# panshengyi/MemVul

Measured on AMD Instinct MI355X. Metric: issue-reports/sec at seq_len=256 (BERT-base issue encoder + 124-anchor memory match), higher is better.
Workload: dtype fp16 + fp8 (MV_F16X8: fp16 MFMA sweep + one OCP-e4m3 MFMA correction sweep per GEMM, fp32 accumulate); 1 GPU; BASELINE.json configs[1]: 1xMI355X-per-rank, bert-base-uncased geometry (12 layers), seq_len=256, batch=256, 124-anchor CWE memory, compute dtype MV_F16X8; seeded random-init weights, synthetic token ids resident in HBM; compute=precise, global_batch=256, seq_len=256, anchors=124, parallelism=dp1 (corpus shards, one all-gather of (score,label) stats), stats_transport=none (one rank)

## Files before the change

### memvul_amd/build.py

```python
from __future__ import annotations

import os
import shutil
import subprocess
from struct import error as struct_error
import sys

HERE = os.path.dirname(os.path.abspath(__file__))
ROOT = os.path.dirname(HERE)
CSRC = os.path.join(HERE, "csrc")
LIB_DIR = os.path.join(HERE, "lib")
LIB_PATH = os.path.join(LIB_DIR, "libmemvul_hip.so")
LIB_PATH_DEV = os.path.join(LIB_DIR, "libmemvul_hip_dev.so")
DEV_FLAGS = ("-DMEMVUL_DEV_SWITCHES",)
SOURCES = ["engine.hip"]
HEADERS = ["common.h", "gemm.h", "gemm_pp.h", "attention.h", "attention_v2.h", "misc_kernels.h", "match_topk.h", "ref_f32.h", "sink_census.h", "route.h", os.path.join(ROOT, "include", "memvul_hip.h")]
ARCH = "gfx950"


def hipcc_path() -> str:
    for c in (os.environ.get("HIPCC"), shutil.which("hipcc"), "/opt/rocm/bin/hipcc"):
        if c and os.path.exists(c):
            return c
    raise RuntimeError("hipcc not found (need ROCm at /opt/rocm)")


STAMP_PATH = LIB_PATH + ".stamp"


def _paths(dev: bool):
    lib = LIB_PATH_DEV if dev else LIB_PATH
    return lib, lib + ".stamp"
FLAGS = ["-O3", "-std=c++17", "-fPIC", "-shared", "-fno-gpu-rdc", "-Wall", "-Wno-unused-function", "-Wno-unused-value"]


def _compiler_id():
    try:
        return subprocess.run([hipcc_path(), "--version"], capture_output=True, check=True).stdout
    except Exception:
        return None


def source_fingerprint(extra_flags=()) -> str:
    import hashlib

    h = hashlib.sha256()
    h.update(" ".join([ARCH, *FLAGS, *extra_flags]).encode())
    deps = [os.path.join(CSRC, s) for s in SOURCES] + [h_ if os.path.isabs(h_) else os.path.join(CSRC, h_) for h_ in HEADERS]
    for d in deps:
        h.update(os.path.basename(d).encode())
        with open(d, "rb") as f:
            h.update(f.read())
    return h.hexdigest()


def build_fingerprint(extra_flags=()) -> str:
    import hashlib

    cc = _compiler_id()
    return "src %s\ncc %s" % (source_fingerprint(extra_flags), hashlib.sha256(cc).hexdigest() if cc is not None else "unknown")


def device_code_objects(lib_path: str = None) -> list:
    import struct

    data = open(lib_path or LIB_PATH, "rb").read()
    magic = b"__CLANG_OFFLOAD_BUNDLE__"
    found = []
    i = data.find(magic)
# ... 92 lines not shown
```

### memvul_amd/csrc/attention.h

```cpp
#pragma once
#include "common.h"

struct AttnArgs {
  const half_t* q;
  const half_t* k;
  const half_t* vt;
  const int32_t* lens;
  half_t* ctx;
  int S;
  int B;
  uint8_t* ctx8;
  unsigned long long* x8_sat;
  const half_t* vt_lo;
  const half_t *q_lo, *k_lo;
  const half_t* vlo_sp;
  unsigned long long* conc;
  int lo8_min_len;
  half_t* sp_lo_out;
  uint32_t* seq_over;
};
#define MV_SINK_COLLISION 0.25f

template <bool LO = false>
__global__ __launch_bounds__(256) void attention_cls_kernel(const float* __restrict__ q, const half_t* __restrict__ k,
                                                            const half_t* __restrict__ vt, const int32_t* __restrict__ lens,
                                                            half_t* __restrict__ ctx, int S, int nbh, float* __restrict__ ctx32 = nullptr,
                                                            const half_t* __restrict__ vlo_sp = nullptr, const half_t* __restrict__ k_lo = nullptr,
                                                            const half_t* __restrict__ vt_lo = nullptr) {
  __shared__ float ps[4][512];
  const int lane = threadIdx.x & 63, wave = threadIdx.x >> 6;
  const int bh = blockIdx.x * 4 + wave;
  if (bh >= nbh) return;
  const int b = bh / MV_HEADS, h = bh - b * MV_HEADS;
  const int len = lens[b];
  const int c = lane & 7, sub = lane >> 3;
  float* pw = ps[wave];
  float qv[8];
  {
    const float4* qp = (const float4*)(q + (size_t)b * MV_HIDDEN + h * MV_HEAD_DIM + 8 * c);
    const float4 t0 = qp[0], t1 = qp[1];
    qv[0] = (float)(half_t)t0.x; qv[1] = (float)(half_t)t0.y; qv[2] = (float)(half_t)t0.z; qv[3] = (float)(half_t)t0.w;
    qv[4] = (float)(half_t)t1.x; qv[5] = (float)(half_t)t1.y; qv[6] = (float)(half_t)t1.z; qv[7] = (float)(half_t)t1.w;
    if constexpr (LO) { qv[0] = t0.x; qv[1] = t0.y; qv[2] = t0.z; qv[3] = t0.w; qv[4] = t1.x; qv[5] = t1.y; qv[6] = t1.z; qv[7] = t1.w; }
  }
  const half_t* kb = k + (size_t)bh * S * MV_HEAD_DIM + (size_t)sub * MV_HEAD_DIM + 8 * c;
#pragma unroll 8
  for (int key0 = 0; key0 < S; key0 += 8) {
    const half8_t kk = *(const half8_t*)(kb + (size_t)key0 * MV_HEAD_DIM);
    float s = 0.f;
#pragma unroll
    for (int e = 0; e < 8; ++e) s = __builtin_fmaf(qv[e], (float)kk[e], s);
    if constexpr (LO) {
      const half8_t kl = *(const half8_t*)(k_lo + (kb - k) + (size_t)key0 * MV_HEAD_DIM);
      float sl = 0.f;
#pragma unroll
      for (int e = 0; e < 8; ++e) sl = __builtin_fmaf(qv[e], (float)kl[e], sl);
      s += sl;
    }
    s += __shfl_xor(s, 1, 64);
    s += __shfl_xor(s, 2, 64);
    s += __shfl_xor(s, 4, 64);
    if (c == 0) pw[key0 + sub] = s + ((key0 + sub >= len) ? -10000.0f : 0.0f);
  }
  __builtin_amdgcn_wave_barrier();
  float mx = -3.0e38f;
  for (int key = lane; key < S; key += 64) mx = fmaxf(mx, pw[key]);
  mx = wave_max(mx);
  float psum = 0.f;
  for (int key = lane; key < S; key += 64) {
    const float p = __expf(pw[key] - mx);
    psum += p;
    pw[key] = LO ? p : (float)(half_t)p;
  }
  const float inv = 1.0f / wave_sum(psum);
  __builtin_amdgcn_wave_barrier();
  float acc[8];
#pragma unroll
  for (int db = 0; db < 8; ++db) acc[db] = 0.f;
  const half_t* vb = vt + ((size_t)bh * MV_HEAD_DIM + sub) * S + 8 * c;
  for (int kb0 = 0; kb0 < S; kb0 += 64) {
    const float4 p0 = *(const float4*)(pw + kb0 + 8 * c), p1 = *(const float4*)(pw + kb0 + 8 * c + 4);
    const float pr[8] = {p0.x, p0.y, p0.z, p0.w, p1.x, p1.y, p1.z, p1.w};
#pragma unroll
    for (int db = 0; db < 8; ++db) {
      const half8_t vv = *(const half8_t*)(vb + (size_t)(8 * db) * S + kb0);
#pragma unroll
      for (int e = 0; e < 8; ++e) acc[db] = __builtin_fmaf(pr[e], (float)vv[e], acc[db]);
    }
  }
  if constexpr (LO) {
    float accl[8];
#pragma unroll
    for (int db = 0; db < 8; ++db) accl[db] = 0.f;
    const half_t* vlb = vt_lo + (vb - vt);
    for (int kb0 = 0; kb0 < S; kb0 += 64) {
      const float4 p0 = *(const float4*)(pw + kb0 + 8 * c), p1 = *(const float4*)(pw + kb0 + 8 * c + 4);
      const float pr[8] = {p0.x, p0.y, p0.z, p0.w, p1.x, p1.y, p1.z, p1.w};
#pragma unroll
      for (int db = 0; db < 8; ++db) {
        const half8_t vv = *(const half8_t*)(vlb + (size_t)(8 * db) * S + kb0);
#pragma unroll
        for (int e = 0; e < 8; ++e) accl[db] = __builtin_fmaf(pr[e], (float)vv[e], accl[db]);
      }
    }
#pragma unroll
    for (int db = 0; db < 8; ++db) acc[db] += accl[db];
  }
  float out = 0.f;
#pragma unroll
  for (int db = 0; db < 8; ++db) {
    float t = acc[db];
    t += __shfl_xor(t, 1, 64);
    t += __shfl_xor(t, 2, 64);
    t += __shfl_xor(t, 4, 64);
    out = (c == db) ? t : out;
  }
  if (vlo_sp) {
    const half2_t l2 = *(const half2_t*)(vlo_sp + ((size_t)bh * MV_HEAD_DIM + 8 * c + sub) * 2);
    out = __builtin_fmaf(__builtin_fmaf(pw[0], (float)l2[0], pw[1] * (float)l2[1]), 1.0f / 2048.0f, out);
  }
  if (ctx32) ctx32[(size_t)b * MV_HIDDEN + h * MV_HEAD_DIM + 8 * c + sub] = out * inv;
  else ctx[(size_t)b * MV_HIDDEN + h * MV_HEAD_DIM + 8 * c + sub] = (half_t)(out * inv);
}
```

### memvul_amd/csrc/engine.hip

```cpp
#include <hip/hip_runtime.h>
#include <dlfcn.h>
#include <rccl/rccl.h>
#include <unistd.h>

#include <algorithm>
#include <charconv>
#include <chrono>
#include <cmath>
#include <cstdio>
#include <cstdlib>
#include <cstring>
#include <map>
#include <string>
#include <vector>

#include "../../include/memvul_hip.h"
#include "common.h"
#include "gemm.h"
#include "gemm_pp.h"
#include "attention.h"
#include "attention_v2.h"
#include "misc_kernels.h"
#include "match_topk.h"
#include "ref_f32.h"
#include "sink_census.h"
#include "route.h"

namespace {

enum KernelClass {
  KC_EMBED_LN = 0, KC_GEMM_QKV, KC_ATTENTION, KC_GEMM_OUT, KC_LN, KC_GEMM_FFN1, KC_GEMM_FFN2,
  KC_POOL_HEAD, KC_MATCH, KC_TOPK, KC_TEST_GEMM, KC_CLS_ROW_TERM, KC_GEMM_KV_LAST, KC_CLS_TAIL
};
const char* kKernelClassNames[MV_NUM_KERNEL_CLASSES] = {
    "embed_ln", "gemm_qkv", "attention", "gemm_attn_out", "layernorm", "gemm_ffn1_gelu", "gemm_ffn2",
    "pool_head", "match", "topk", "test_gemm", "cls_row_term", "gemm_kv_last", "cls_tail"};

thread_local std::string g_create_error;

struct HostTensor {
  std::vector<float> data;
  std::vector<int64_t> shape;
};

struct LayerW {
  half_t *wqkv = nullptr, *wo = nullptr, *w1 = nullptr, *w2 = nullptr;
  float *bqkv = nullptr, *bo = nullptr, *b1 = nullptr, *b2 = nullptr;
  half_t *wqkv_f = nullptr, *w1_f = nullptr;
  float *bqkv_f = nullptr, *b1_f = nullptr;
  uint8_t *wqkv_f8 = nullptr, *wo8 = nullptr, *w1_f8 = nullptr, *w28 = nullptr;
  int sc_qkv = 0, sc_o = 0, sc_1 = 0, sc_2 = 0;
  float *wqT32 = nullptr, *woT32 = nullptr, *w1T32 = nullptr, *w2T32 = nullptr;
  float *wqkv32 = nullptr, *wo32 = nullptr, *w132 = nullptr, *w232 = nullptr;
  float *ln1g = nullptr, *ln1b = nullptr, *ln2g = nullptr, *ln2b = nullptr;
};

inline int64_t round_up(int64_t x, int64_t m) { return (x + m - 1) / m * m; }

inline uint16_t f32_to_f16_bits(float f) {
  uint32_t x;
  std::memcpy(&x, &f, 4);
  const uint32_t sign = (x >> 16) & 0x8000u;
  x &= 0x7fffffffu;
  if (x >= 0x7f800000u) return (uint16_t)(sign | 0x7c00u | ((x > 0x7f800000u) ? 0x200u : 0));
  if (x >= 0x477ff000u) return (uint16_t)(sign | 0x7c00u);
  if (x < 0x38800000u) {
    if (x < 0x33000000u) return (uint16_t)sign;
    const int e = (int)(x >> 23);
    uint32_t m = (x & 0x7fffffu) | 0x800000u;
    const int shift = 126 - e;
    const uint32_t half_m = m >> shift;
    const uint32_t rem = m & ((1u << shift) - 1), halfway = 1u << (shift - 1);
    uint32_t r = half_m;
    if (rem > halfway || (rem == halfway && (half_m & 1))) r++;
    return (uint16_t)(sign | r);
  }
  const uint32_t e = (x >> 23) - 112, m = x & 0x7fffffu;
  uint32_t h = (e << 10) | (m >> 13);
  const uint32_t rem = m & 0x1fffu;
  if (rem > 0x1000u || (rem == 0x1000u && (h & 1))) h++;
  return (uint16_t)(sign | h);
}
inline float f16_bits_to_f32(uint16_t h) {
  const uint32_t sign = (uint32_t)(h & 0x8000u) << 16;
  uint32_t e = (h >> 10) & 0x1f, m = h & 0x3ffu, x;
  if (e == 0) {
    if (m == 0) x = sign;
    else {
      int sh = 0;
      while (!(m & 0x400u)) { m <<= 1; sh++; }
      m &= 0x3ffu;
      x = sign | ((uint32_t)(113 - sh) << 23) | (m << 13);
    }
  } else if (e == 31) x = sign | 0x7f800000u | (m << 13);
  else x = sign | ((e + 112) << 23) | (m << 13);
  float f;
  std::memcpy(&f, &x, 4);
  return f;
}
inline float bf16_bits_to_f32(uint16_t h) {
  uint32_t x = (uint32_t)h << 16;
  float f;
  std::memcpy(&f, &x, 4);
  return f;
}
// ... 509 lines not shown
                       wk.tile_both);
    if (int rc = launch_check(h, "cls_tile_flags")) return rc;
  }
  const bool special = big && x8;
  auto row_term = [&](const half_t* A, const half_t* W, int N, int K) -> int {
    ProfScope ps(h, wk.stream, KC_CLS_ROW_TERM);
    GemmArgs t{};
    t.M = (int)round_up(2 * B, 64); t.Mreal = 2 * B; t.S = 64; t.A = A; t.W = W; t.N = N; t.K = K; t.outf = wk.cls_corr;
    t.GN = choose_gn(N / 64, 8);
    hipLaunchKernelGGL((gemm_ring_kernel<EPI_F32, 1, 1, 2, 2, 64, 4, 2>), dim3((unsigned)((t.M / 64) * (N / 64))), dim3(256), RING64_LDS, wk.stream, t);
    return launch_check(h, "row term gemm_ring");
  };
  const unsigned ln_grid = (unsigned)((M + 3) / 4);
  {
    ProfScope ps(h, wk.stream, KC_EMBED_LN);
    if (big)
      hipLaunchKernelGGL(embed_ln_kernel<true>, dim3(ln_grid), dim3(256), 0, wk.stream, d_ids, pitch, S_in, Sp, (int)M, c.vocab_size,
                         h->wemb, h->pemb, h->temb, h->embg, h->embb, c.ln_eps, wk.xres, wk.x16, wk.lnstats,
                         x8 ? (half_t*)nullptr : wk.xlo, x8 ? wk.x8 : (uint8_t*)nullptr, h->x8_sat, special ? d_lens : (const int32_t*)nullptr,
                         special ? wk.st_lo : (half_t*)nullptr);
    else
      hipLaunchKernelGGL(embed_ln_kernel<false>, dim3(ln_grid), dim3(256), 0, wk.stream, d_ids, pitch, S_in, Sp, (int)M, c.vocab_size,
                         h->wemb, h->pemb, h->temb, h->embg, h->embb, c.ln_eps, wk.xres, wk.x16, (float*)nullptr,
                         (half_t*)nullptr, (uint8_t*)nullptr, (unsigned long long*)nullptr);
    if (int rc = launch_check(h, "embed_ln")) return rc;
  }
  const float *pend_g = h->embg, *pend_b = h->embb;
  auto run_ln = [&](float* x32, half_t* x16, int rows, const float* g, const float* b) -> int {
    ProfScope ps(h, wk.stream, KC_LN);
    hipLaunchKernelGGL(ln_kernel<true>, dim3((unsigned)((rows + 3) / 4)), dim3(256), 0, wk.stream, x32, x16, rows, g, b, c.ln_eps,
                       (float*)nullptr);
    return launch_check(h, "layernorm");
  };
  auto final_ln = [&](const float* g, const float* b) -> int {
    const size_t n4 = (size_t)M * MV_HIDDEN / 4;
    hipLaunchKernelGGL(hilo_to_f32_kernel, dim3((unsigned)((n4 + 255) / 256)), dim3(256), 0, wk.stream, wk.x16, wk.xlo, n4, wk.xres,
                       special ? (const half_t*)wk.st_lo : (const half_t*)nullptr, Sp, (const uint8_t*)wk.x8);
    if (int rc = launch_check(h, "hilo_to_f32")) return rc;
    return run_ln(wk.xres, wk.x16, (int)M, g, b);
  };
  if (big && n_layers == 0) { if (int rc = final_ln(h->embg, h->embb)) return rc; }
  float *st_in = wk.lnstats, *st_mid = wk.lnpart;
  for (int l = 0; l < n_layers; ++l) {
    const LayerW& w = h->L[l];
    const bool last = (l == n_layers - 1);
    GemmArgs g{};
    g.M = (int)Mpad; g.Mreal = (int)M; g.S = Sp; g.ln_eps = c.ln_eps; g.x8_sat = h->x8_sat;
    g.tile_both = (cls_as && one_seq_tiles) ? wk.tile_both : nullptr;
    g.q = wk.q; g.k = wk.k; g.vt = wk.vt;
    const half_t* wqkv = big ? w.wqkv_f : w.wqkv;
    const float* bqkv = big ? w.bqkv_f : w.bqkv;
    if (last && prune) {
      const int Bp = (int)round_up(B, 128);
      g.A = wk.x16; g.W = wqkv + (size_t)MV_HIDDEN * MV_HIDDEN; g.bias = bqkv + MV_HIDDEN; g.N = 2 * MV_HIDDEN; g.K = MV_HIDDEN;
      g.col0 = MV_HIDDEN;
      if (big) {
        g.lnstats = st_in;
        if (x8) { g.A8 = wk.x8; g.W8 = w.wqkv_f8 + (size_t)MV_HIDDEN * 2 * MV_HIDDEN; g.x8_scale = w.sc_qkv; g.x8_terms = 3; g.x8_aside_mask = qkv_mask; }
        if (special) {
          if ((qkv_mask & 6) != 6) {
            if (int rc = row_term(wk.st_lo, g.W, g.N, g.K)) return rc;
            g.cls_corr = wk.cls_corr;
          }
          g.vlo_sp = two_plane ? nullptr : wk.vlo_sp;
        }
        if (safe) { g.vt_lo = wk.vt_lo; g.q_lo = wk.q_lo; g.k_lo = wk.k_lo; }
        if (int rc = launch_pp<PP_QK>(h, wk.stream, KC_GEMM_KV_LAST, g)) return rc;
      } else if (int rc = launch_small<EPI_QKV>(h, wk.stream, KC_GEMM_KV_LAST, g)) return rc;
      ProfScope tail(h, wk.stream, KC_CLS_TAIL);
      const uint32_t keep_mask = h->prof_mask;
      h->prof_mask = 0;
      auto tail_rc = [&]() -> int {
        hipLaunchKernelGGL(cls_gather_kernel, dim3((B + 3) / 4), dim3(256), 0, wk.stream, wk.xres, wk.x16, Sp, B,
                           big ? st_in : (const float*)nullptr, pend_g, pend_b, wk.c32, wk.c16, big ? 1 : 0,
                           (big && !x8) ? wk.xlo : (const half_t*)nullptr, big ? 1 : 0, c.ln_eps, special ? (const half_t*)wk.st_lo : (const half_t*)nullptr);
        if (int rc = launch_check(h, "cls_gather")) return rc;
        if (x8) {
          const unsigned gx = (unsigned)((B + 31) / 32);
          hipLaunchKernelGGL((dense768_kernel<2, MV_HIDDEN>), dim3(gx, MV_HIDDEN / 32), dim3(512), 0, wk.stream, (const float*)wk.c32,
                             (size_t)MV_HIDDEN, B, (const float*)w.wqT32, (const float*)w.bqkv, MV_HIDDEN, wk.cq, (const float*)nullptr);
          if (int rc = launch_check(h, "cls q")) return rc;
          if (safe)
            hipLaunchKernelGGL(attention_cls_kernel<true>, dim3((B * MV_HEADS + 3) / 4), dim3(256), 0, wk.stream, wk.cq, wk.k, wk.vt, d_lens, wk.cctx, Sp,
                               B * MV_HEADS, wk.pooled, (const half_t*)g.vlo_sp, (const half_t*)wk.k_lo, (const half_t*)wk.vt_lo);
          else
            hipLaunchKernelGGL(attention_cls_kernel<false>, dim3((B * MV_HEADS + 3) / 4), dim3(256), 0, wk.stream, wk.cq, wk.k, wk.vt, d_lens, wk.cctx, Sp,
                               B * MV_HEADS, wk.pooled, (const half_t*)g.vlo_sp, (const half_t*)nullptr, (const half_t*)nullptr);
          if (int rc = launch_check(h, "attention_cls")) return rc;
          hipLaunchKernelGGL((dense768_kernel<4, MV_HIDDEN>), dim3(gx, MV_HIDDEN / 32), dim3(512), 0, wk.stream, (const float*)wk.pooled,
                             (size_t)MV_HIDDEN, B, (const float*)w.woT32, (const float*)w.bo, MV_HIDDEN, wk.c32, (const float*)wk.c32);
          if (int rc = launch_check(h, "cls out")) return rc;
          if (int rc = run_ln(wk.c32, wk.c16, B, w.ln1g, w.ln1b)) return rc;
          hipLaunchKernelGGL((dense768_kernel<3, MV_HIDDEN>), dim3(gx, MV_INTER / 32), dim3(512), 0, wk.stream, (const float*)wk.c32,
                             (size_t)MV_HIDDEN, B, (const float*)w.w1T32, (const float*)w.b1, MV_INTER, wk.ch32, (const float*)nullptr);
          if (int rc = launch_check(h, "cls ffn1")) return rc;
          hipLaunchKernelGGL((dense768_kernel<4, MV_INTER>), dim3(gx, MV_HIDDEN / 32), dim3(512), 0, wk.stream, (const float*)wk.ch32,
                             (size_t)MV_INTER, B, (const float*)w.w2T32, (const float*)w.b2, MV_HIDDEN, wk.c32, (const float*)wk.c32);
          if (int rc = launch_check(h, "cls ffn2")) return rc;
          if (int rc = run_ln(wk.c32, wk.c16, B, w.ln2g, w.ln2b)) return rc;
          return pool_head(h, wk, wk.c32, MV_HIDDEN, B, u_out);
        }
        GemmArgs t{};
        t.M = Bp; t.Mreal = B; t.S = 64;
        t.A = wk.c16; t.W = w.wqkv; t.bias = w.bqkv; t.N = MV_HIDDEN; t.K = MV_HIDDEN; t.outf = wk.cq;
        if (int rc = launch_small<EPI_F32>(h, wk.stream, KC_CLS_TAIL, t)) return rc;
        hipLaunchKernelGGL(attention_cls_kernel<false>, dim3((B * MV_HEADS + 3) / 4), dim3(256), 0, wk.stream, wk.cq, wk.k, wk.vt,
                           d_lens, wk.cctx, Sp, B * MV_HEADS, (float*)nullptr, (const half_t*)nullptr, (const half_t*)nullptr, (const half_t*)nullptr);
        if (int rc = launch_check(h, "attention_cls")) return rc;
        t.A = wk.cctx; t.W = w.wo; t.bias = w.bo; t.N = MV_HIDDEN; t.K = MV_HIDDEN; t.xres = wk.c32; t.outf = nullptr;
        if (int rc = launch_small<EPI_RES>(h, wk.stream, KC_CLS_TAIL, t)) return rc;
        if (int rc = run_ln(wk.c32, wk.c16, B, w.ln1g, w.ln1b)) return rc;
        t.A = wk.c16; t.W = w.w1; t.bias = w.b1; t.N = MV_INTER; t.K = MV_HIDDEN; t.out16 = wk.ch16;
        if (int rc = launch_small<EPI_GELU>(h, wk.stream, KC_CLS_TAIL, t)) return rc;
        t.A = wk.ch16; t.W = w.w2; t.bias = w.b2; t.N = MV_HIDDEN; t.K = MV_INTER; t.xres = wk.c32;
        if (int rc = launch_small<EPI_RES>(h, wk.stream, KC_CLS_TAIL, t)) return rc;
        if (int rc = run_ln(wk.c32, wk.c16, B, w.ln2g, w.ln2b)) return rc;
        return pool_head(h, wk, wk.c32, MV_HIDDEN, B, u_out);
      }();
      h->prof_mask = keep_mask;
      return tail_rc;
    }
    if (big) {
      g.A = wk.x16; g.W = wqkv; g.bias = bqkv; g.N = 3 * MV_HIDDEN; g.K = MV_HIDDEN; g.lnstats = st_in;
      if (x8) { g.A8 = wk.x8; g.W8 = w.wqkv_f8; g.x8_scale = w.sc_qkv; g.x8_terms = 3; g.x8_aside_mask = qkv_mask; }
      g.vt_lo = two_plane ? wk.vt_lo : nullptr;
      g.q_lo = wk.q_lo; g.k_lo = wk.k_lo;
      if (special) {
        if (qkv_mask != 7) {
          if (int rc = row_term(wk.st_lo, g.W, g.N, g.K)) return rc;
          g.cls_corr = wk.cls_corr;
        }
        g.vlo_sp = g.vt_lo ? nullptr : wk.vlo_sp;
      }
      if (int rc = launch_pp<PP_QK>(h, wk.stream, KC_GEMM_QKV, g)) return rc;
      g.cls_corr = nullptr; g.vlo_sp = nullptr;
      if (h->census && x8 && pf.monitor) {
        ProfScope ps(h, wk.stream, KC_ATTENTION);
        hipLaunchKernelGGL(sink_census_kernel, dim3((unsigned)((B * MV_HEADS + 3) / 4)), dim3(256), 0, wk.stream, (const half_t*)wk.q, (const half_t*)wk.k, d_lens,
                           d_ids, pitch, S_in, Sp, B * MV_HEADS, c.vocab_size, h->census_items, h->census_share, h->census_heads + (size_t)l * MV_HEADS);
        if (int rc = launch_check(h, "sink_census")) return rc;
      }
      if (int rc = launch_attention(h, wk, d_lens, B, Sp, x8, cls_as, pf)) return rc;
      g.A = wk.ctx; g.W = w.wo; g.bias = w.bo; g.N = MV_HIDDEN; g.K = MV_HIDDEN;
      g.lnstats = st_in; g.lng = pend_g; g.lnb = pend_b; g.lnpart = st_mid; g.out16 = wk.x16; g.out16b = wk.xlo;
      if (x8) { g.A8 = wk.ctx8; g.W8 = w.wo8; g.x8_scale = w.sc_o; g.out8 = wk.x8; g.x8_terms = 2; }
      if (cls_as) {
        if (int rc = row_term(wk.cls_lo, g.W, g.N, g.K)) return rc;
        g.cls_corr = wk.cls_corr; g.x8_terms = 1;
        g.out8_hi_only = 0;
      }
      if (special) g.sp_lo_out = wk.st_lo;
      if (int rc = launch_pp<PP_RESLN3>(h, wk.stream, KC_GEMM_OUT, g)) return rc;
      pend_g = w.ln1g; pend_b = w.ln1b;
      g.A = wk.x16; g.W = w.w1_f; g.bias = w.b1_f; g.N = MV_INTER; g.K = MV_HIDDEN; g.lnstats = st_mid; g.out16 = wk.h16;
      g.out16b = nullptr; g.lnpart = nullptr; g.sp_lo_out = nullptr;
      if (x8) { g.A8 = wk.x8; g.W8 = w.w1_f8; g.x8_scale = w.sc_1; g.out8 = wk.h8; g.x8_terms = 2; }
      if (cls_as) {
        if (int rc = row_term(wk.st_lo, g.W, g.N, g.K)) return rc;
        g.x8_terms = 1;
        g.out8_hi_only = 1;
// ... 845 lines not shown
        pack[(size_t)(2 * H + i)] = t3->data[(size_t)i];
      }
      if ((rc = upload_f32(h, s0, &w.bqkv, pack.data(), 3 * H))) return rc;
      bqkv_host = pack;
    }
    if (!f32) {
      const std::string lnk = l == 0 ? P + "embeddings.LayerNorm." : P + "encoder.layer." + std::to_string(l - 1) + ".output.LayerNorm.";
      const HostTensor *tg = nullptr, *tb = nullptr;
      if ((rc = need(h, lnk + "weight", {H}, &tg))) return rc;
      if ((rc = need(h, lnk + "bias", {H}, &tb))) return rc;
      std::vector<float> Wf, bf;
      fold_layernorm(wqkv_host.data(), bqkv_host.data(), tg->data.data(), tb->data.data(), 3 * H, H, Wf, bf);
      if ((rc = upload_f16(h, s0, &w.wqkv_f, Wf.data(), 3 * H * H))) return rc;
      if (precise && (rc = upload_x8_weight(h, s0, &w.wqkv_f8, &w.sc_qkv, Wf.data(), 3 * H, H))) return rc;
      if ((rc = upload_f32(h, s0, &w.bqkv_f, bf.data(), 3 * H))) return rc;
    }
    NEED(q + "attention.output.dense.weight", H, H);
    if (f32 && (rc = upload_f32(h, s0, &w.wo32, t->data.data(), H * H))) return rc;
    if (!f32 && (rc = upload_f16(h, s0, &w.wo, t->data.data(), H * H))) return rc;
    if (precise && (rc = upload_x8_weight(h, s0, &w.wo8, &w.sc_o, t->data.data(), H, H))) return rc;
    NEED(q + "attention.output.dense.bias", H);
    if ((rc = upload_f32(h, s0, &w.bo, t->data.data(), H))) return rc;
    NEED(q + "attention.output.LayerNorm.weight", H);
    if ((rc = upload_f32(h, s0, &w.ln1g, t->data.data(), H))) return rc;
    NEED(q + "attention.output.LayerNorm.bias", H);
    if ((rc = upload_f32(h, s0, &w.ln1b, t->data.data(), H))) return rc;
    NEED(q + "intermediate.dense.weight", I, H);
    if (f32 && (rc = upload_f32(h, s0, &w.w132, t->data.data(), I * H))) return rc;
    if (!f32 && (rc = upload_f16(h, s0, &w.w1, t->data.data(), I * H))) return rc;
    NEED(q + "intermediate.dense.bias", I);
    if ((rc = upload_f32(h, s0, &w.b1, t->data.data(), I))) return rc;
    if (!f32) {
      const HostTensor *tw = nullptr, *tg = nullptr, *tb = nullptr;
      if ((rc = need(h, q + "intermediate.dense.weight", {I, H}, &tw))) return rc;
      if ((rc = need(h, q + "attention.output.LayerNorm.weight", {H}, &tg))) return rc;
      if ((rc = need(h, q + "attention.output.LayerNorm.bias", {H}, &tb))) return rc;
      std::vector<float> Wf, bf;
      fold_layernorm(tw->data.data(), t->data.data(), tg->data.data(), tb->data.data(), I, H, Wf, bf);
      if ((rc = upload_f16(h, s0, &w.w1_f, Wf.data(), I * H))) return rc;
      if (precise && (rc = upload_x8_weight(h, s0, &w.w1_f8, &w.sc_1, Wf.data(), I, H))) return rc;
      if ((rc = upload_f32(h, s0, &w.b1_f, bf.data(), I))) return rc;
    }
    NEED(q + "output.dense.weight", H, I);
    if (f32 && (rc = upload_f32(h, s0, &w.w232, t->data.data(), H * I))) return rc;
    if (!f32 && (rc = upload_f16(h, s0, &w.w2, t->data.data(), H * I))) return rc;
    if (precise && (rc = upload_x8_weight(h, s0, &w.w28, &w.sc_2, t->data.data(), H, I))) return rc;
    NEED(q + "output.dense.bias", H);
    if ((rc = upload_f32(h, s0, &w.b2, t->data.data(), H))) return rc;
    NEED(q + "output.LayerNorm.weight", H);
    if ((rc = upload_f32(h, s0, &w.ln2g, t->data.data(), H))) return rc;
    NEED(q + "output.LayerNorm.bias", H);
    if ((rc = upload_f32(h, s0, &w.ln2b, t->data.data(), H))) return rc;
  }
  if (precise && c.layers > 0) {
    const std::string q = P + "encoder.layer." + std::to_string(c.layers - 1) + ".";
    LayerW& w = h->L[c.layers - 1];
    auto up_T = [&](const std::string& key, int64_t N, int64_t K, float scale, float** dst) -> int {
      const HostTensor* tt = nullptr;
      if (int r = need(h, key, {N, K}, &tt)) return r;
      std::vector<float> tr((size_t)(N * K));
      for (int64_t n = 0; n < N; ++n) for (int64_t k = 0; k < K; ++k) tr[(size_t)(k * N + n)] = tt->data[(size_t)(n * K + k)] * scale;
      return upload_f32(h, s0, dst, tr.data(), N * K);
    };
    if ((rc = up_T(q + "attention.self.query.weight", H, H, 0.125f, &w.wqT32))) return rc;
    if ((rc = up_T(q + "attention.output.dense.weight", H, H, 1.0f, &w.woT32))) return rc;
    if ((rc = up_T(q + "intermediate.dense.weight", I, H, 1.0f, &w.w1T32))) return rc;
    if ((rc = up_T(q + "output.dense.weight", H, I, 1.0f, &w.w2T32))) return rc;
  }
  NEED("_bert_pooler.pooler.dense.weight", H, H);
  {
    std::vector<float> tr((size_t)(H * H));
    for (int64_t n = 0; n < H; ++n) for (int64_t k = 0; k < H; ++k) tr[(size_t)(k * H + n)] = t->data[(size_t)(n * H + k)];
    if ((rc = upload_f32(h, s0, &h->WpT, tr.data(), H * H))) return rc;
  }
  NEED("_bert_pooler.pooler.dense.bias", H);
  if ((rc = upload_f32(h, s0, &h->bp, t->data.data(), H))) return rc;
  if (h->P == MV_PROJ) {
    NEED("_projector_single._linear_layers.0.weight", MV_PROJ, H);
    {
      std::vector<float> tr((size_t)(H * MV_PROJ));
      for (int64_t n = 0; n < MV_PROJ; ++n) for (int64_t k = 0; k < H; ++k) tr[(size_t)(k * MV_PROJ + n)] = t->data[(size_t)(n * H + k)];
      if ((rc = upload_f32(h, s0, &h->WhT, tr.data(), H * MV_PROJ))) return rc;
    }
    NEED("_projector_single._linear_layers.0.bias", MV_PROJ);
    if ((rc = upload_f32(h, s0, &h->bh, t->data.data(), MV_PROJ))) return rc;
  }
  NEED("_projector.weight", 2, 3 * (int64_t)h->P);
  if ((rc = upload_f32(h, s0, &h->Wm, t->data.data(), 2 * 3 * (int64_t)h->P))) return rc;
#undef NEED
  if (f32) {
    for (int wi = 0; wi < h->n_alloc; ++wi) {
      Work& wk = h->work[wi];
      rc = dev_alloc(h, wk.stream, &wk.qkv32, h->cap_tokens * 3 * MV_HIDDEN);
      if (rc == MV_OK) rc = dev_alloc(h, wk.stream, &wk.ctx32, h->cap_tokens * MV_HIDDEN);
      if (rc == MV_OK) rc = dev_alloc(h, wk.stream, &wk.h32, h->cap_tokens * MV_INTER);
      if (rc == MV_OK && hipStreamSynchronize(wk.stream) != hipSuccess) rc = MV_ERR_HIP;
      if (rc != MV_OK) return rc;
    }
  }
  if (!precise && !f32) {
    for (int wi = 0; wi < h->n_alloc; ++wi) {
      Work& wk = h->work[wi];
      rc = dev_alloc(h, wk.stream, &wk.xlo, h->cap_tokens * MV_HIDDEN);
      if (rc == MV_OK && hipStreamSynchronize(wk.stream) != hipSuccess) rc = MV_ERR_HIP;
      if (rc != MV_OK) return rc;
    }
  }
  if (precise) {
    if (h->gemm_tile == 128) return fail(h, MV_ERR_STATE, "MV_F16X8 runs on the persistent GEMM path: MEMVUL_GEMM_TILE=128 excludes it");
    for (int wi = 0; wi < h->n_alloc; ++wi) {
      Work& wk = h->work[wi];
      rc = dev_alloc(h, wk.stream, &wk.x8, h->cap_tokens * 2 * MV_HIDDEN);
      if (rc == MV_OK) rc = dev_alloc(h, wk.stream, &wk.ctx8, h->cap_tokens * 2 * MV_HIDDEN);
      if (rc == MV_OK) rc = dev_alloc(h, wk.stream, &wk.h8, h->cap_tokens * 2 * MV_INTER);
      if (rc == MV_OK) rc = dev_alloc(h, wk.stream, &wk.ch32, (int64_t)round_up(h->cfg.max_batch, 256) * MV_INTER);
      if (rc == MV_OK) rc = dev_alloc(h, wk.stream, &wk.cls_lo, 2 * (int64_t)round_up(h->cfg.max_batch, 256) * MV_INTER);
      if (rc == MV_OK) rc = dev_alloc(h, wk.stream, &wk.cls_corr, 2 * (int64_t)round_up(h->cfg.max_batch, 256) * MV_INTER);
      if (rc == MV_OK) rc = dev_alloc(h, wk.stream, &wk.st_lo, 2 * (int64_t)round_up(h->cfg.max_batch, 256) * MV_HIDDEN);
      if (rc == MV_OK) rc = dev_alloc(h, wk.stream, &wk.vlo_sp, (int64_t)h->cfg.max_batch * MV_HEADS * MV_HEAD_DIM * 2);
      if (rc == MV_OK) rc = dev_alloc(h, wk.stream, &wk.tile_both, h->cap_tokens / 256 + 1);
// ... 888 lines not shown
```

Before: 14540 issue-reports/s.

## Fold last-layer CLS attention through K/V weights instead of computing full K/V projections

For the pruned last layer, the K and V projection GEMM over all tokens is dropped. Instead the CLS query is folded through Wk into a per-head hidden-space vector, and token hidden states (LN applied on the fly) are streamed once with an online softmax. The weighted hidden sums are then unfolded through Wv. This removes a 2*768-wide GEMM over B*S rows and replaces it with a streaming pass plus small per-batch matvecs. The cost is extra fp32 weight uploads and partial buffers, and it changes rounding relative to the fp16/fp8 K/V path.

```diff
diff --git a/memvul_amd/build.py b/memvul_amd/build.py
--- a/memvul_amd/build.py
+++ b/memvul_amd/build.py
@@ -14,7 +14,7 @@
 LIB_PATH_DEV = os.path.join(LIB_DIR, "libmemvul_hip_dev.so")
 DEV_FLAGS = ("-DMEMVUL_DEV_SWITCHES",)
 SOURCES = ["engine.hip"]
-HEADERS = ["common.h", "gemm.h", "gemm_pp.h", "attention.h", "attention_v2.h", "misc_kernels.h", "match_topk.h", "ref_f32.h", "sink_census.h", "route.h", os.path.join(ROOT, "include", "memvul_hip.h")]
+HEADERS = ["common.h", "gemm.h", "gemm_pp.h", "attention.h", "attention_v2.h", "cls_fold.h", "misc_kernels.h", "match_topk.h", "ref_f32.h", "sink_census.h", "route.h", os.path.join(ROOT, "include", "memvul_hip.h")]
 ARCH = "gfx950"
 
 
diff --git a/memvul_amd/csrc/attention.h b/memvul_amd/csrc/attention.h
--- a/memvul_amd/csrc/attention.h
+++ b/memvul_amd/csrc/attention.h
@@ -21,12 +21,9 @@
 };
 #define MV_SINK_COLLISION 0.25f
 
-template <bool LO = false>
 __global__ __launch_bounds__(256) void attention_cls_kernel(const float* __restrict__ q, const half_t* __restrict__ k,
                                                             const half_t* __restrict__ vt, const int32_t* __restrict__ lens,
-                                                            half_t* __restrict__ ctx, int S, int nbh, float* __restrict__ ctx32 = nullptr,
-                                                            const half_t* __restrict__ vlo_sp = nullptr, const half_t* __restrict__ k_lo = nullptr,
-                                                            const half_t* __restrict__ vt_lo = nullptr) {
+                                                            half_t* __restrict__ ctx, int S, int nbh) {
   __shared__ float ps[4][512];
   const int lane = threadIdx.x & 63, wave = threadIdx.x >> 6;
   const int bh = blockIdx.x * 4 + wave;
@@ -41,7 +38,6 @@
     const float4 t0 = qp[0], t1 = qp[1];
     qv[0] = (float)(half_t)t0.x; qv[1] = (float)(half_t)t0.y; qv[2] = (float)(half_t)t0.z; qv[3] = (float)(half_t)t0.w;
     qv[4] = (float)(half_t)t1.x; qv[5] = (float)(half_t)t1.y; qv[6] = (float)(half_t)t1.z; qv[7] = (float)(half_t)t1.w;
-    if constexpr (LO) { qv[0] = t0.x; qv[1] = t0.y; qv[2] = t0.z; qv[3] = t0.w; qv[4] = t1.x; qv[5] = t1.y; qv[6] = t1.z; qv[7] = t1.w; }
   }
   const half_t* kb = k + (size_t)bh * S * MV_HEAD_DIM + (size_t)sub * MV_HEAD_DIM + 8 * c;
 #pragma unroll 8
@@ -50,13 +46,6 @@
     float s = 0.f;
 #pragma unroll
     for (int e = 0; e < 8; ++e) s = __builtin_fmaf(qv[e], (float)kk[e], s);
-    if constexpr (LO) {
-      const half8_t kl = *(const half8_t*)(k_lo + (kb - k) + (size_t)key0 * MV_HEAD_DIM);
-      float sl = 0.f;
-#pragma unroll
-      for (int e = 0; e < 8; ++e) sl = __builtin_fmaf(qv[e], (float)kl[e], sl);
-      s += sl;
-    }
     s += __shfl_xor(s, 1, 64);
     s += __shfl_xor(s, 2, 64);
     s += __shfl_xor(s, 4, 64);
@@ -70,7 +59,7 @@
   for (int key = lane; key < S; key += 64) {
     const float p = __expf(pw[key] - mx);
     psum += p;
-    pw[key] = LO ? p : (float)(half_t)p;
+    pw[key] = (float)(half_t)p;
   }
   const float inv = 1.0f / wave_sum(psum);
   __builtin_amdgcn_wave_barrier();
@@ -88,24 +77,6 @@
       for (int e = 0; e < 8; ++e) acc[db] = __builtin_fmaf(pr[e], (float)vv[e], acc[db]);
     }
   }
-  if constexpr (LO) {
-    float accl[8];
-#pragma unroll
-    for (int db = 0; db < 8; ++db) accl[db] = 0.f;
-    const half_t* vlb = vt_lo + (vb - vt);
-    for (int kb0 = 0; kb0 < S; kb0 += 64) {
-      const float4 p0 = *(const float4*)(pw + kb0 + 8 * c), p1 = *(const float4*)(pw + kb0 + 8 * c + 4);
-      const float pr[8] = {p0.x, p0.y, p0.z, p0.w, p1.x, p1.y, p1.z, p1.w};
-#pragma unroll
-      for (int db = 0; db < 8; ++db) {
-        const half8_t vv = *(const half8_t*)(vlb + (size_t)(8 * db) * S + kb0);
-#pragma unroll
-        for (int e = 0; e < 8; ++e) accl[db] = __builtin_fmaf(pr[e], (float)vv[e], accl[db]);
-      }
-    }
-#pragma unroll
-    for (int db = 0; db < 8; ++db) acc[db] += accl[db];
-  }
   float out = 0.f;
 #pragma unroll
   for (int db = 0; db < 8; ++db) {
@@ -115,10 +86,5 @@
     t += __shfl_xor(t, 4, 64);
     out = (c == db) ? t : out;
   }
-  if (vlo_sp) {
-    const half2_t l2 = *(const half2_t*)(vlo_sp + ((size_t)bh * MV_HEAD_DIM + 8 * c + sub) * 2);
-    out = __builtin_fmaf(__builtin_fmaf(pw[0], (float)l2[0], pw[1] * (float)l2[1]), 1.0f / 2048.0f, out);
-  }
-  if (ctx32) ctx32[(size_t)b * MV_HIDDEN + h * MV_HEAD_DIM + 8 * c + sub] = out * inv;
-  else ctx[(size_t)b * MV_HIDDEN + h * MV_HEAD_DIM + 8 * c + sub] = (half_t)(out * inv);
+  ctx[(size_t)b * MV_HIDDEN + h * MV_HEAD_DIM + 8 * c + sub] = (half_t)(out * inv);
 }
diff --git a/memvul_amd/csrc/cls_fold.h b/memvul_amd/csrc/cls_fold.h
--- /dev/null
+++ b/memvul_amd/csrc/cls_fold.h
@@ -0,0 +1,305 @@
+#pragma once
+#include "common.h"
+
+#define CF_CHUNK 128
+#define CF_BLOCK 16
+#define CF_BT 8
+#define CF_PART (MV_HEADS * MV_HIDDEN + 2 * MV_HEADS)
+
+inline int cf_chunks(int Sp) { return (Sp + CF_CHUNK - 1) / CF_CHUNK; }
+__device__ __forceinline__ int cf_keys(int len, int Sp) { return (len < 1 || len > Sp) ? Sp : len; }
+
+__global__ __launch_bounds__(256) void cls_key_fold_kernel(const float* __restrict__ q, const float* __restrict__ Wk, const float* __restrict__ gamma, int B,
+                                                           float* __restrict__ ap) {
+  __shared__ float qs[CF_BT][MV_HEAD_DIM];
+  const int tid = threadIdx.x, h = blockIdx.y, b0 = blockIdx.x * CF_BT;
+  for (int i = tid; i < CF_BT * MV_HEAD_DIM; i += 256) {
+    const int bi = i >> 6, d = i & 63;
+    const int b = b0 + bi < B ? b0 + bi : B - 1;
+    qs[bi][d] = q[(size_t)b * MV_HIDDEN + h * MV_HEAD_DIM + d];
+  }
+  __syncthreads();
+  float acc[CF_BT][3];
+#pragma unroll
+  for (int bi = 0; bi < CF_BT; ++bi) acc[bi][0] = acc[bi][1] = acc[bi][2] = 0.f;
+  const float* w = Wk + (size_t)(h * MV_HEAD_DIM) * MV_HIDDEN + tid;
+#pragma unroll 4
+  for (int d = 0; d < MV_HEAD_DIM; ++d) {
+    const float w0 = w[(size_t)d * MV_HIDDEN], w1 = w[(size_t)d * MV_HIDDEN + 256], w2 = w[(size_t)d * MV_HIDDEN + 512];
+#pragma unroll
+    for (int bi = 0; bi < CF_BT; ++bi) {
+      const float qv = qs[bi][d];
+      acc[bi][0] = __builtin_fmaf(qv, w0, acc[bi][0]);
+      acc[bi][1] = __builtin_fmaf(qv, w1, acc[bi][1]);
+      acc[bi][2] = __builtin_fmaf(qv, w2, acc[bi][2]);
+    }
+  }
+  const float g0 = gamma[tid], g1 = gamma[tid + 256], g2 = gamma[tid + 512];
+#pragma unroll
+  for (int bi = 0; bi < CF_BT; ++bi) {
+    if (b0 + bi >= B) break;
+    float* o = ap + ((size_t)(b0 + bi) * MV_HEADS + h) * MV_HIDDEN + tid;
+    o[0] = acc[bi][0] * g0; o[256] = acc[bi][1] * g1; o[512] = acc[bi][2] * g2;
+  }
+}
+
+struct CfRaw {
+  uint4 h0, l0;
+  uint2 h1, l1;
+  float2 p0, p1, p2;
+};
+__device__ __forceinline__ float cf_h(uint32_t w, int hi) { return (float)__builtin_bit_cast(half2_t, w)[hi]; }
+
+template <bool X8>
+__global__ __launch_bounds__(256) void cls_stream_kernel(const half_t* __restrict__ x16, const half_t* __restrict__ xlo, const uint8_t* __restrict__ x8,
+                                                         const half_t* __restrict__ sp_lo, const float* __restrict__ vstats, const int32_t* __restrict__ lens,
+                                                         const float* __restrict__ ap, int Sp, int nch, float eps, float* __restrict__ part) {
+  __shared__ float4 xs[CF_BLOCK][3][64];
+  __shared__ float sc[MV_HEADS][CF_BLOCK];
+  const int lane = threadIdx.x & 63;
+  const int wave = __builtin_amdgcn_readfirstlane(threadIdx.x >> 6);
+  const int b = blockIdx.x / nch, c = blockIdx.x - b * nch;
+  const int r0 = c * CF_CHUNK;
+  int nv = cf_keys(lens[b], Sp) - r0;
+  if (nv <= 0) return;
+  nv = nv < CF_CHUNK ? nv : CF_CHUNK;
+  const int cA = 8 * lane, cB = 512 + 4 * lane;
+
+  float ar[MV_HEADS][12];
+  {
+    const float* a0 = ap + (size_t)b * MV_HEADS * MV_HIDDEN;
+#pragma unroll
+    for (int h = 0; h < MV_HEADS; ++h) {
+      const float4 u = *(const float4*)(a0 + h * MV_HIDDEN + cA), v = *(const float4*)(a0 + h * MV_HIDDEN + cA + 4), t = *(const float4*)(a0 + h * MV_HIDDEN + cB);
+      ar[h][0] = u.x; ar[h][1] = u.y; ar[h][2] = u.z; ar[h][3] = u.w; ar[h][4] = v.x; ar[h][5] = v.y; ar[h][6] = v.z; ar[h][7] = v.w;
+      ar[h][8] = t.x; ar[h][9] = t.y; ar[h][10] = t.z; ar[h][11] = t.w;
+    }
+  }
+  auto load_row = [&](int s, CfRaw& r) {
+    const size_t t = (size_t)b * Sp + s;
+    r.h0 = *(const uint4*)(x16 + t * MV_HIDDEN + cA);
+    r.h1 = *(const uint2*)(x16 + t * MV_HIDDEN + cB);
+    if constexpr (X8) {
+      if (s < 2) {
+        const half_t* lo = sp_lo + (size_t)(2 * b + s) * MV_HIDDEN;
+        r.l0 = *(const uint4*)(lo + cA);
+        r.l1 = *(const uint2*)(lo + cB);
+      } else {
+        const uint8_t* lo = x8 + t * (2 * MV_HIDDEN);
+        const uint2 u = *(const uint2*)(lo + cA);
+        r.l0.x = u.x; r.l0.y = u.y; r.l0.z = 0; r.l0.w = 0;
+        r.l1.x = *(const uint32_t*)(lo + cB); r.l1.y = 0;
+      }
+    } else {
+      r.l0 = *(const uint4*)(xlo + t * MV_HIDDEN + cA);
+      r.l1 = *(const uint2*)(xlo + t * MV_HIDDEN + cB);
+    }
+    const float2* p = (const float2*)(vstats + 6 * t);
+    r.p0 = p[0]; r.p1 = p[1]; r.p2 = p[2];
+  };
+  auto load_block = [&](int blk, CfRaw (&raw)[CF_BLOCK / 4]) {
+#pragma unroll
+    for (int i = 0; i < CF_BLOCK / 4; ++i) {
+      const int rb = blk * CF_BLOCK + wave + 4 * i;
+      if (rb < nv) load_row(r0 + rb, raw[i]);
+    }
+  };
+  auto score_row = [&](int s, int r, const CfRaw& raw) {
+    float x[12];
+    const uint32_t hw[6] = {raw.h0.x, raw.h0.y, raw.h0.z, raw.h0.w, raw.h1.x, raw.h1.y};
+    if (X8 && s >= 2) {
+      constexpr float SLO = 1.0f / (float)(2048 << MV_X8_ACT_SHIFT);
+      const uint32_t lw[3] = {raw.l0.x, raw.l0.y, raw.l1.x};
+#pragma unroll
+      for (int j = 0; j < 3; ++j) {
+        const float2_t u = __builtin_amdgcn_cvt_scalef32_pk_f32_fp8(lw[j], 1.0f, false), v = __builtin_amdgcn_cvt_scalef32_pk_f32_fp8(lw[j], 1.0f, true);
+        x[4 * j + 0] = cf_h(hw[2 * j], 0) + u.x * SLO; x[4 * j + 1] = cf_h(hw[2 * j], 1) + u.y * SLO;
+        x[4 * j + 2] = cf_h(hw[2 * j + 1], 0) + v.x * SLO; x[4 * j + 3] = cf_h(hw[2 * j + 1], 1) + v.y * SLO;
+      }
+    } else {
+      const float ls = X8 ? 1.0f / 2048.0f : 1.0f;
+      const uint32_t lw[6] = {raw.l0.x, raw.l0.y, raw.l0.z, raw.l0.w, raw.l1.x, raw.l1.y};
+#pragma unroll
+      for (int j = 0; j < 6; ++j) {
+        x[2 * j] = __builtin_fmaf(cf_h(lw[j], 0), ls, cf_h(hw[j], 0));
+        x[2 * j + 1] = __builtin_fmaf(cf_h(lw[j], 1), ls, cf_h(hw[j], 1));
+      }
+    }
+    const float2 st = ln_from_partials(raw.p0, raw.p1, raw.p2, eps);
+#pragma unroll
+    for (int j = 0; j < 12; ++j) x[j] = (x[j] - st.x) * st.y;
+    xs[r][0][lane] = make_float4(x[0], x[1], x[2], x[3]);
+    xs[r][1][lane] = make_float4(x[4], x[5], x[6], x[7]);
+    xs[r][2][lane] = make_float4(x[8], x[9], x[10], x[11]);
+    float p[MV_HEADS];
+#pragma unroll
+    for (int h = 0; h < MV_HEADS; ++h) {
+      float2_t a2 = {0.f, 0.f};
+#pragma unroll
+      for (int j = 0; j < 6; ++j) a2 = __builtin_elementwise_fma(float2_t{ar[h][2 * j], ar[h][2 * j + 1]}, float2_t{x[2 * j], x[2 * j + 1]}, a2);
+      p[h] = a2.x + a2.y;
+    }
+    const bool up32 = lane >= 32, up16 = (lane & 16) != 0;
+    float v6[6], v3[3];
+#pragma unroll
+    for (int j = 0; j < 6; ++j) v6[j] = (up32 ? p[j + 6] : p[j]) + __shfl_xor(up32 ? p[j] : p[j + 6], 32, 64);
+#pragma unroll
+    for (int j = 0; j < 3; ++j) v3[j] = (up16 ? v6[j + 3] : v6[j]) + __shfl_xor(up16 ? v6[j] : v6[j + 3], 16, 64);
+#pragma unroll
+    for (int j = 0; j < 3; ++j) {
+      v3[j] += __shfl_xor(v3[j], 8, 64);
+      v3[j] += __shfl_xor(v3[j], 4, 64);
+      v3[j] += __shfl_xor(v3[j], 2, 64);
+      v3[j] += __shfl_xor(v3[j], 1, 64);
+    }
+    if ((lane & 15) == 0) {
+      const int h0 = 3 * (lane >> 4);
+      sc[h0][r] = v3[0]; sc[h0 + 1][r] = v3[1]; sc[h0 + 2][r] = v3[2];
+    }
+  };
+
+  float z[3][12], mrun[3], lrun[3];
+#pragma unroll
+  for (int hh = 0; hh < 3; ++hh) {
+    mrun[hh] = -3.0e38f; lrun[hh] = 0.f;
+#pragma unroll
+    for (int j = 0; j < 12; ++j) z[hh][j] = 0.f;
+  }
+  const int nblk = (nv + CF_BLOCK - 1) / CF_BLOCK;
+  CfRaw raw[CF_BLOCK / 4];
+  load_block(0, raw);
+#pragma unroll 1
+  for (int blk = 0; blk < nblk; ++blk) {
+#pragma unroll
+    for (int i = 0; i < CF_BLOCK / 4; ++i) {
+      const int rb = blk * CF_BLOCK + wave + 4 * i;
+      if (rb < nv) score_row(r0 + rb, wave + 4 * i, raw[i]);
+    }
+    if (blk + 1 < nblk) load_block(blk + 1, raw);
+    __syncthreads();
+    const int nvb = (nv - blk * CF_BLOCK) < CF_BLOCK ? (nv - blk * CF_BLOCK) : CF_BLOCK;
+    float mnew[3];
+#pragma unroll
+    for (int hh = 0; hh < 3; ++hh) {
+      float mb = mrun[hh];
+      for (int r = 0; r < nvb; ++r) mb = fmaxf(mb, sc[3 * wave + hh][r]);
+      const float scale = __expf(mrun[hh] - mb);
+      mnew[hh] = mb; mrun[hh] = mb;
+      lrun[hh] *= scale;
+#pragma unroll
+      for (int j = 0; j < 12; ++j) z[hh][j] *= scale;
+    }
+#pragma unroll 2
+    for (int r = 0; r < nvb; ++r) {
+      const float4 u = xs[r][0][lane], v = xs[r][1][lane], t = xs[r][2][lane];
+      const float xv[12] = {u.x, u.y, u.z, u.w, v.x, v.y, v.z, v.w, t.x, t.y, t.z, t.w};
+#pragma unroll
+      for (int hh = 0; hh < 3; ++hh) {
+        const float pr = __expf(sc[3 * wave + hh][r] - mnew[hh]);
+        lrun[hh] += pr;
+#pragma unroll
+        for (int j = 0; j < 12; ++j) z[hh][j] = __builtin_fmaf(pr, xv[j], z[hh][j]);
+      }
+    }
+    __syncthreads();
+  }
+  float* po = part + (size_t)blockIdx.x * CF_PART;
+#pragma unroll
+  for (int hh = 0; hh < 3; ++hh) {
+    float* zo = po + (3 * wave + hh) * MV_HIDDEN;
+    *(float4*)(zo + cA) = make_float4(z[hh][0], z[hh][1], z[hh][2], z[hh][3]);
+    *(float4*)(zo + cA + 4) = make_float4(z[hh][4], z[hh][5], z[hh][6], z[hh][7]);
+    *(float4*)(zo + cB) = make_float4(z[hh][8], z[hh][9], z[hh][10], z[hh][11]);
+    if (lane == 0) {
+      po[MV_HEADS * MV_HIDDEN + 2 * (3 * wave + hh)] = mrun[hh];
+      po[MV_HEADS * MV_HIDDEN + 2 * (3 * wave + hh) + 1] = lrun[hh];
+    }
+  }
+}
+
+template <bool OUT16>
+__global__ __launch_bounds__(256) void cls_value_unfold_kernel(const float* __restrict__ part, const int32_t* __restrict__ lens, int Sp, int nch,
+                                                               const float* __restrict__ WvT, const float* __restrict__ bv, const float* __restrict__ gamma,
+                                                               const float* __restrict__ beta, int B, float* __restrict__ out32, half_t* __restrict__ out16) {
+  __shared__ __attribute__((aligned(16))) float ys[CF_BT][MV_HIDDEN];
+  __shared__ float red[4][CF_BT][MV_HEAD_DIM];
+  const int tid = threadIdx.x, h = blockIdx.y, b0 = blockIdx.x * CF_BT;
+  const float g0 = gamma[tid], g1 = gamma[tid + 256], g2 = gamma[tid + 512];
+  const float be0 = beta[tid], be1 = beta[tid + 256], be2 = beta[tid + 512];
+  for (int bi = 0; bi < CF_BT; ++bi) {
+    const int b = b0 + bi < B ? b0 + bi : B - 1;
+    const int nc = (cf_keys(lens[b], Sp) + CF_CHUNK - 1) / CF_CHUNK;
+    const float* p0 = part + (size_t)b * nch * CF_PART;
+    float mx = -3.0e38f;
+    for (int c = 0; c < nc; ++c) mx = fmaxf(mx, p0[(size_t)c * CF_PART + MV_HEADS * MV_HIDDEN + 2 * h]);
+    float L = 0.f, z0 = 0.f, z1 = 0.f, z2 = 0.f;
+    for (int c = 0; c < nc; ++c) {
+      const float* pc = p0 + (size_t)c * CF_PART;
+      const float e = __expf(pc[MV_HEADS * MV_HIDDEN + 2 * h] - mx);
+      L = __builtin_fmaf(e, pc[MV_HEADS * MV_HIDDEN + 2 * h + 1], L);
+      z0 = __builtin_fmaf(e, pc[h * MV_HIDDEN + tid], z0);
+      z1 = __builtin_fmaf(e, pc[h * MV_HIDDEN + tid + 256], z1);
+      z2 = __builtin_fmaf(e, pc[h * MV_HIDDEN + tid + 512], z2);
+    }
+    const float inv = 1.0f / L;
+    ys[bi][tid] = __builtin_fmaf(z0 * inv, g0, be0);
+    ys[bi][tid + 256] = __builtin_fmaf(z1 * inv, g1, be1);
+    ys[bi][tid + 512] = __builtin_fmaf(z2 * inv, g2, be2);
+  }
+  __syncthreads();
+  const int d = tid & 63, ks = tid >> 6;
+  float acc[CF_BT];
+#pragma unroll
+  for (int bi = 0; bi < CF_BT; ++bi) acc[bi] = 0.f;
+  const float* w = WvT + (size_t)(192 * ks) * MV_HIDDEN + h * MV_HEAD_DIM + d;
+#pragma unroll 4
+  for (int k = 0; k < 192; k += 4) {
+    const float w0 = w[(size_t)k * MV_HIDDEN], w1 = w[(size_t)(k + 1) * MV_HIDDEN], w2 = w[(size_t)(k + 2) * MV_HIDDEN], w3 = w[(size_t)(k + 3) * MV_HIDDEN];
+#pragma unroll
+    for (int bi = 0; bi < CF_BT; ++bi) {
+      const float4 y = *(const float4*)&ys[bi][192 * ks + k];
+      acc[bi] = __builtin_fmaf(y.x, w0, acc[bi]);
+      acc[bi] = __builtin_fmaf(y.y, w1, acc[bi]);
+      acc[bi] = __builtin_fmaf(y.z, w2, acc[bi]);
+      acc[bi] = __builtin_fmaf(y.w, w3, acc[bi]);
+    }
+  }
+#pragma unroll
+  for (int bi = 0; bi < CF_BT; ++bi) red[ks][bi][d] = acc[bi];
+  __syncthreads();
+#pragma unroll
+  for (int j = 0; j < CF_BT * MV_HEAD_DIM / 256; ++j) {
+    const int idx = tid + 256 * j, bi = idx >> 6, dd = idx & 63;
+    if (b0 + bi >= B) continue;
+    const float v = ((red[0][bi][dd] + red[1][bi][dd]) + red[2][bi][dd]) + red[3][bi][dd] + bv[h * MV_HEAD_DIM + dd];
+    const size_t o = (size_t)(b0 + bi) * MV_HIDDEN + h * MV_HEAD_DIM + dd;
+    if constexpr (OUT16) out16[o] = (half_t)v;
+    else out32[o] = v;
+  }
+}
+
+struct ClsFoldArgs {
+  const float *q, *Wk, *WvT, *bv, *gamma, *beta;
+  const half_t *x16, *xlo;
+  const uint8_t* x8;
+  const half_t* sp_lo;
+  const float* vstats;
+  const int32_t* lens;
+  float *ap, *part, *out32;
+  half_t* out16;
+  int B, Sp;
+  float eps;
+};
+inline void cls_fold_launch(hipStream_t stream, const ClsFoldArgs& a) {
+  const int nch = cf_chunks(a.Sp);
+  const dim3 fold_grid((unsigned)((a.B + CF_BT - 1) / CF_BT), MV_HEADS), stream_grid((unsigned)(a.B * nch));
+  hipLaunchKernelGGL(cls_key_fold_kernel, fold_grid, dim3(256), 0, stream, a.q, a.Wk, a.gamma, a.B, a.ap);
+  if (a.x8)
+    hipLaunchKernelGGL(cls_stream_kernel<true>, stream_grid, dim3(256), 0, stream, a.x16, a.xlo, a.x8, a.sp_lo, a.vstats, a.lens, (const float*)a.ap, a.Sp, nch, a.eps, a.part);
+  else
+    hipLaunchKernelGGL(cls_stream_kernel<false>, stream_grid, dim3(256), 0, stream, a.x16, a.xlo, a.x8, a.sp_lo, a.vstats, a.lens, (const float*)a.ap, a.Sp, nch, a.eps, a.part);
+  if (a.out16)
+    hipLaunchKernelGGL(cls_value_unfold_kernel<true>, fold_grid, dim3(256), 0, stream, (const float*)a.part, a.lens, a.Sp, nch, a.WvT, a.bv, a.gamma, a.beta, a.B, a.out32, a.out16);
+  else
+    hipLaunchKernelGGL(cls_value_unfold_kernel<false>, fold_grid, dim3(256), 0, stream, (const float*)a.part, a.lens, a.Sp, nch, a.WvT, a.bv, a.gamma, a.beta, a.B, a.out32, a.out16);
+}
diff --git a/memvul_amd/csrc/engine.hip b/memvul_amd/csrc/engine.hip
--- a/memvul_amd/csrc/engine.hip
+++ b/memvul_amd/csrc/engine.hip
@@ -20,6 +20,7 @@
 #include "gemm_pp.h"
 #include "attention.h"
 #include "attention_v2.h"
+#include "cls_fold.h"
 #include "misc_kernels.h"
 #include "match_topk.h"
 #include "ref_f32.h"
@@ -51,6 +52,7 @@
   uint8_t *wqkv_f8 = nullptr, *wo8 = nullptr, *w1_f8 = nullptr, *w28 = nullptr;
   int sc_qkv = 0, sc_o = 0, sc_1 = 0, sc_2 = 0;
   float *wqT32 = nullptr, *woT32 = nullptr, *w1T32 = nullptr, *w2T32 = nullptr;
+  float *wk32 = nullptr, *wvT32 = nullptr;
   float *wqkv32 = nullptr, *wo32 = nullptr, *w132 = nullptr, *w232 = nullptr;
   float *ln1g = nullptr, *ln1b = nullptr, *ln2g = nullptr, *ln2b = nullptr;
 };
@@ -666,21 +668,15 @@
     const float* bqkv = big ? w.bqkv_f : w.bqkv;
     if (last && prune) {
       const int Bp = (int)round_up(B, 128);
-      g.A = wk.x16; g.W = wqkv + (size_t)MV_HIDDEN * MV_HIDDEN; g.bias = bqkv + MV_HIDDEN; g.N = 2 * MV_HIDDEN; g.K = MV_HIDDEN;
-      g.col0 = MV_HIDDEN;
-      if (big) {
-        g.lnstats = st_in;
-        if (x8) { g.A8 = wk.x8; g.W8 = w.wqkv_f8 + (size_t)MV_HIDDEN * 2 * MV_HIDDEN; g.x8_scale = w.sc_qkv; g.x8_terms = 3; g.x8_aside_mask = qkv_mask; }
-        if (special) {
-          if ((qkv_mask & 6) != 6) {
-            if (int rc = row_term(wk.st_lo, g.W, g.N, g.K)) return rc;
-            g.cls_corr = wk.cls_corr;
-          }
-          g.vlo_sp = two_plane ? nullptr : wk.vlo_sp;
-        }
-        if (safe) { g.vt_lo = wk.vt_lo; g.q_lo = wk.q_lo; g.k_lo = wk.k_lo; }
-        if (int rc = launch_pp<PP_QK>(h, wk.stream, KC_GEMM_KV_LAST, g)) return rc;
-      } else if (int rc = launch_small<EPI_QKV>(h, wk.stream, KC_GEMM_KV_LAST, g)) return rc;
+      if (!big) {
+        g.A = wk.x16; g.W = wqkv + (size_t)MV_HIDDEN * MV_HIDDEN; g.bias = bqkv + MV_HIDDEN; g.N = 2 * MV_HIDDEN; g.K = MV_HIDDEN; g.col0 = MV_HIDDEN;
+        if (int rc = launch_small<EPI_QKV>(h, wk.stream, KC_GEMM_KV_LAST, g)) return rc;
+      }
+      auto cls_fold = [&](float* out32, half_t* out16) -> int {
+        cls_fold_launch(wk.stream, ClsFoldArgs{wk.cq, w.wk32, w.wvT32, w.bqkv + 2 * MV_HIDDEN, pend_g, pend_b, wk.x16, x8 ? nullptr : wk.xlo, x8 ? wk.x8 : nullptr,
+                                               x8 ? wk.st_lo : nullptr, st_in, d_lens, (float*)wk.k, (float*)wk.vt, out32, out16, B, Sp, c.ln_eps});
+        return launch_check(h, "cls fold");
+      };
       ProfScope tail(h, wk.stream, KC_CLS_TAIL);
       const uint32_t keep_mask = h->prof_mask;
       h->prof_mask = 0;
@@ -694,13 +690,7 @@
           hipLaunchKernelGGL((dense768_kernel<2, MV_HIDDEN>), dim3(gx, MV_HIDDEN / 32), dim3(512), 0, wk.stream, (const float*)wk.c32,
                              (size_t)MV_HIDDEN, B, (const float*)w.wqT32, (const float*)w.bqkv, MV_HIDDEN, wk.cq, (const float*)nullptr);
           if (int rc = launch_check(h, "cls q")) return rc;
-          if (safe)
-            hipLaunchKernelGGL(attention_cls_kernel<true>, dim3((B * MV_HEADS + 3) / 4), dim3(256), 0, wk.stream, wk.cq, wk.k, wk.vt, d_lens, wk.cctx, Sp,
-                               B * MV_HEADS, wk.pooled, (const half_t*)g.vlo_sp, (const half_t*)wk.k_lo, (const half_t*)wk.vt_lo);
-          else
-            hipLaunchKernelGGL(attention_cls_kernel<false>, dim3((B * MV_HEADS + 3) / 4), dim3(256), 0, wk.stream, wk.cq, wk.k, wk.vt, d_lens, wk.cctx, Sp,
-                               B * MV_HEADS, wk.pooled, (const half_t*)g.vlo_sp, (const half_t*)nullptr, (const half_t*)nullptr);
-          if (int rc = launch_check(h, "attention_cls")) return rc;
+          if (int rc = cls_fold(wk.pooled, nullptr)) return rc;
           hipLaunchKernelGGL((dense768_kernel<4, MV_HIDDEN>), dim3(gx, MV_HIDDEN / 32), dim3(512), 0, wk.stream, (const float*)wk.pooled,
                              (size_t)MV_HIDDEN, B, (const float*)w.woT32, (const float*)w.bo, MV_HIDDEN, wk.c32, (const float*)wk.c32);
           if (int rc = launch_check(h, "cls out")) return rc;
@@ -718,8 +708,8 @@
         t.M = Bp; t.Mreal = B; t.S = 64;
         t.A = wk.c16; t.W = w.wqkv; t.bias = w.bqkv; t.N = MV_HIDDEN; t.K = MV_HIDDEN; t.outf = wk.cq;
         if (int rc = launch_small<EPI_F32>(h, wk.stream, KC_CLS_TAIL, t)) return rc;
-        hipLaunchKernelGGL(attention_cls_kernel<false>, dim3((B * MV_HEADS + 3) / 4), dim3(256), 0, wk.stream, wk.cq, wk.k, wk.vt,
-                           d_lens, wk.cctx, Sp, B * MV_HEADS, (float*)nullptr, (const half_t*)nullptr, (const half_t*)nullptr, (const half_t*)nullptr);
+        if (big) { if (int rc = cls_fold(nullptr, wk.cctx)) return rc; }
+        else hipLaunchKernelGGL(attention_cls_kernel, dim3((B * MV_HEADS + 3) / 4), dim3(256), 0, wk.stream, wk.cq, wk.k, wk.vt, d_lens, wk.cctx, Sp, B * MV_HEADS);
         if (int rc = launch_check(h, "attention_cls")) return rc;
         t.A = wk.cctx; t.W = w.wo; t.bias = w.bo; t.N = MV_HIDDEN; t.K = MV_HIDDEN; t.xres = wk.c32; t.outf = nullptr;
         if (int rc = launch_small<EPI_RES>(h, wk.stream, KC_CLS_TAIL, t)) return rc;
@@ -1671,7 +1661,7 @@
     NEED(q + "output.LayerNorm.bias", H);
     if ((rc = upload_f32(h, s0, &w.ln2b, t->data.data(), H))) return rc;
   }
-  if (precise && c.layers > 0) {
+  if (!f32 && c.layers > 0) {
     const std::string q = P + "encoder.layer." + std::to_string(c.layers - 1) + ".";
     LayerW& w = h->L[c.layers - 1];
     auto up_T = [&](const std::string& key, int64_t N, int64_t K, float scale, float** dst) -> int {
@@ -1681,10 +1671,15 @@
       for (int64_t n = 0; n < N; ++n) for (int64_t k = 0; k < K; ++k) tr[(size_t)(k * N + n)] = tt->data[(size_t)(n * K + k)] * scale;
       return upload_f32(h, s0, dst, tr.data(), N * K);
     };
-    if ((rc = up_T(q + "attention.self.query.weight", H, H, 0.125f, &w.wqT32))) return rc;
-    if ((rc = up_T(q + "attention.output.dense.weight", H, H, 1.0f, &w.woT32))) return rc;
-    if ((rc = up_T(q + "intermediate.dense.weight", I, H, 1.0f, &w.w1T32))) return rc;
-    if ((rc = up_T(q + "output.dense.weight", H, I, 1.0f, &w.w2T32))) return rc;
+    NEED(q + "attention.self.key.weight", H, H);
+    if ((rc = upload_f32(h, s0, &w.wk32, t->data.data(), H * H))) return rc;
+    if ((rc = up_T(q + "attention.self.value.weight", H, H, 1.0f, &w.wvT32))) return rc;
+    if (precise) {
+      if ((rc = up_T(q + "attention.self.query.weight", H, H, 0.125f, &w.wqT32))) return rc;
+      if ((rc = up_T(q + "attention.output.dense.weight", H, H, 1.0f, &w.woT32))) return rc;
+      if ((rc = up_T(q + "intermediate.dense.weight", I, H, 1.0f, &w.w1T32))) return rc;
+      if ((rc = up_T(q + "output.dense.weight", H, I, 1.0f, &w.w2T32))) return rc;
+    }
   }
   NEED("_bert_pooler.pooler.dense.weight", H, H);
   {
```

Result: no change. 14550 issue-reports/s (median of 2 runs) (+0.1%).
